# cv-core/MIT-Driverless-CV-TrainingInfra

Hardware: AMD Instinct MI355X
Metric: images/sec training (YOLOv3 416^2 + RektNet 80^2) (higher is better)
Workload: dtype bf16; 1 GPU; CVC-YOLOv3 yolo_baseline 416x416 classes=80, train step (fwd+bwd+Adam), 32 img/GPU; global_batch=32, parallelism=dp1, hipgraph=False, optimizer=FusedAdam

## Files before the change

include/mdcv_hip.h:

```cpp
#ifndef MDCV_HIP_H
#define MDCV_HIP_H
#ifdef __cplusplus
extern "C" {
#endif

#define MDCV_OK 0
#define MDCV_EARG (-1)
#define MDCV_F32 0
#define MDCV_BF16 1
#define MDCV_TUNED(dtype, code) (((dtype) & 0xff) | ((code) * 256))
#define MDCV_ACT_NONE 0
#define MDCV_ACT_LEAKY 1
#define MDCV_ACT_RELU 2

int mdcv_conv2d(int dtype, int mode, const void* in, int in_ldc, const void* w_packed, void* out, int out_ldc,
                const float* bias, const void* addsrc, int add_ldc, float* stats_partial,
                int B, int Hin, int Win, int Cin, int Hout, int Wout, int Nout,
                int KH, int KW, int stride, int pad, int dil, void* stream);
int mdcv_conv2d_affine_act(int dtype, const void* in, int in_ldc, const void* w_packed, void* out, int out_ldc, const float* scale,
                           const float* shift, const void* addsrc, int add_ldc, int act, float slope, int B, int Hin, int Win, int Cin,
                           int Hout, int Wout, int Nout, int KH, int KW, int stride, int pad, int dil, void* stream);
int mdcv_conv2d_dgrad_bnsums_rows(int dtype, int B, int Hin, int Win, int Cin, int Hout, int Wout, int Nout, int KH, int KW, int stride,
                                  int pad, int dil, int in_ldc);
int mdcv_conv2d_dgrad_bnsums(int dtype, const void* in, int in_ldc, const void* w_packed, void* out, int out_ldc, const void* addsrc,
                             int add_ldc, int B, int Hin, int Win, int Cin, int Hout, int Wout, int Nout, int KH, int KW, int stride,
                             int pad, int dil, const void* y, int ldy, const float* scale, const float* shift, const float* mean, int act,
                             float slope, float* partial, void* stream);
int mdcv_first_conv_ok(int dtype, int B, int H, int W, int Cin_pad, int Cout_pad, int KH, int KW, int stride, int pad, int dil, int ldx);
int mdcv_first_conv_rows(int B, int H);
int mdcv_first_conv_stats(int dtype, const void* x, int ldx, const void* w_packed, float* partial, int B, int H, int W, void* stream);
int mdcv_first_conv_bn_act(int dtype, const void* x, int ldx, const void* w_packed, const float* scale, const float* shift, int act, float slope,
                           void* y, int ldy, void* z, int ldz, int B, int H, int W, void* stream);
int mdcv_conv2d_dgrad_s2_form_ok(int dtype, int B, int Hin, int Win, int Cin, int Hout, int Wout, int Nout, int KH, int KW, int stride,
                                 int pad, int dil, int in_ldc);
int mdcv_xstats_words(int reps, int C);
int mdcv_xstats_reps(int rows, int C);
int mdcv_conv2d_xstats(int dtype, const void* in, int in_ldc, const void* w_packed, void* out, int out_ldc, const float* bias, void* xacc,
                       int reps, int B, int Hin, int Win, int Cin, int Hout, int Wout, int Nout, int KH, int KW, int stride, int pad, int dil,
                       void* stream);
int mdcv_pw_conv_fwd_xstats(int dtype, const void* y, int ldy, const float* scale, const float* shift, const void* resid, int ldr, int act,
                            float slope, void* z_out, int ldz, const void* w_packed, const float* bias, void* out, int out_ldc, void* xacc,
                            int reps, long long M, int K, int N, void* stream);
int mdcv_bn_act_fwd_xstats(int dtype, const void* y, int ldy, const void* xacc, int reps, double count, const float* gamma, const float* beta,
                           float* running_mean, float* running_var, float momentum, float eps, float* scale, float* shift, float* mean,
                           float* invstd, const void* resid, int ldr, void* out, int ldo, int M, int C, int act, float slope, void* stream);
int mdcv_conv2d_stats_rows(int M);
int mdcv_conv2d_stats_rows_geom(int dtype, int B, int Hout, int Wout, int Cin, int Nout, int KH, int KW, int stride, int pad, int dil,
                                int in_ldc);

int mdcv_conv2d_wgrad_splits(int dtype, int M, int Cout, int Ktot);
int mdcv_conv2d_wgrad_splits_geom(int dtype, int B, int Hin, int Win, int Cin, int Hout, int Wout, int Cout, int KH, int KW, int stride,
                                  int pad, int dil, int dy_ldc, int x_ldc);
int mdcv_conv2d_wgrad(int dtype, const void* dy, int dy_ldc, const void* x, int x_ldc, float* ws, int splits,
                      float* dw_oihw, int accumulate, int B, int Hin, int Win, int Cin, int Cin_real,
                      int Hout, int Wout, int Cout, int Cout_real, int KH, int KW, int stride, int pad, int dil, void* stream);

int mdcv_pack_weights(int dtype, const float* w_oihw, void* w_fwd, void* w_dgrad, int Cout, int Cin, int KH, int KW,
                      int Cout_pad, int Cin_pad, void* stream);

int mdcv_pack_weights_batched(int dtype, const void* table, int nlayers, int max_taps, void* stream);

int mdcv_nchw_to_nhwc(int dtype, const float* src, void* dst, int B, int C, int H, int W, int ldc, int Cpad, void* stream);
int mdcv_nhwc_to_nchw(int dtype, const void* src, int ldc, float* dst, int B, int C, int H, int W, void* stream);

int mdcv_partial_reduce(const float* partial, int rows, int nsums, int C, double* accum, void* stream);
int mdcv_bn_finalize(double* accum, double count, const float* gamma, const float* beta, float* running_mean, float* running_var,
                     float momentum, float eps, float* scale, float* shift, float* mean, float* invstd, int C, void* stream);
// ... 174 lines not shown
```

mit-driverless-cv-traininginfra_amd/csrc/conv_igemm.hip:

```cpp
#include "conv_gemm.h"
#include "conv_shift.h"
#include "wgrad_gemm.h"
#include "wgrad_shift.h"
#include "wgrad_stream.h"

extern "C" {

static int conv2d_impl(int dtype, int mode, const void* in, int in_ldc, const void* w_packed, void* out, int out_ldc,
                       const float* bias, const void* addsrc, int add_ldc, float* stats_partial,
                       int B, int Hin, int Win, int Cin, int Hout, int Wout, int Nout,
                       int KH, int KW, int stride, int pad, int dil, const BnFuseArgs* fuse, void* stream, const EpiArgs* epi = nullptr,
                       const XAccArgs* xacc = nullptr) {
  if (!in || !w_packed || !out) return MDCV_EARG;
  if (xacc && (mode != 0 || stats_partial || fuse || epi || !xacc->acc || xacc->reps < 1 || (xacc->reps & (xacc->reps - 1)))) return MDCV_EARG;
  if (epi && (mode != 0 || stats_partial || fuse)) return MDCV_EARG;
  if ((Cin & 7) || (Nout & 7) || (in_ldc & 7) || (out_ldc & 7) || (addsrc && (add_ldc & 7))) return MDCV_EARG;
  if (stride != 1 && stride != 2) return MDCV_EARG;
  if (mode != 0 && mode != 1) return MDCV_EARG;
  ConvArgs a;
  a.in = in; a.w = w_packed; a.out = out; a.bias = bias; a.addsrc = addsrc; a.stats = stats_partial;
  a.in_ldc = in_ldc; a.out_ldc = out_ldc; a.add_ldc = add_ldc;
  a.Hin = Hin; a.Win = Win; a.Cin = Cin; a.Hout = Hout; a.Wout = Wout; a.Nout = Nout;
  a.KH = KH; a.KW = KW; a.stride = stride; a.pad = pad; a.dil = dil;
  a.M = B * Hout * Wout; a.Ktot = KH * KW * Cin; a.tiles_n = 0; a.sshift = stride == 2 ? 1 : 0; a.tiles_total = 0; a.xcd_chunk = 0;
// ... 105 lines not shown
    int rows = 0;
    for (int cls = 0; cls < 4; ++cls) {
      const int ph = cls >> 1, pw = cls & 1;
      const int m = B * ((Hout - ph + 1) / 2) * ((Wout - pw + 1) / 2);
      if (m > 0) rows += cdiv(m, 128);
    }
    return rows;
  }
  return cdiv(B * Hout * Wout, 128);
}

int mdcv_conv2d_dgrad_bnsums(int dtype, const void* in, int in_ldc, const void* w_packed, void* out, int out_ldc, const void* addsrc,
                             int add_ldc, int B, int Hin, int Win, int Cin, int Hout, int Wout, int Nout, int KH, int KW, int stride,
                             int pad, int dil, const void* y, int ldy, const float* scale, const float* shift, const float* mean, int act,
                             float slope, float* partial, void* stream) {
  MDCV_TUNE_ENTRY(dtype, MDCV_TUNE_CONV);
  if (!y || !scale || !shift || !mean || !partial || (ldy & 7)) return MDCV_EARG;
  if (mdcv_conv2d_dgrad_bnsums_rows(dtype, B, Hin, Win, Cin, Hout, Wout, Nout, KH, KW, stride, pad, dil, in_ldc) <= 0) return MDCV_EARG;
  BnFuseArgs f;
  f.y = y; f.scale = scale; f.shift = shift; f.mean = mean; f.partial = partial; f.ldy = ldy; f.act = act; f.row_base = 0;
  f.slope = act == 2 ? 0.f : slope;
  return conv2d_impl(dtype, 1, in, in_ldc, w_packed, out, out_ldc, nullptr, addsrc, add_ldc, nullptr, B, Hin, Win, Cin, Hout, Wout, Nout,
                     KH, KW, stride, pad, dil, &f, stream);
}

int mdcv_conv2d_dgrad_s2_form_ok(int dtype, int B, int Hin, int Win, int Cin, int Hout, int Wout, int Nout, int KH, int KW, int stride,
                                 int pad, int dil, int in_ldc) {
  MDCV_TUNE_ENTRY(dtype, MDCV_TUNE_CONV);
  return dtype == MDCV_BF16 && stride == 2 && dil == 1 && KH == 3 && KW == 3 && pad == 1 && Hout == 2 * Hin && Wout == 2 * Win &&
         TUNE().conv_variant < 0 && (long long)B * Hin * Win * in_ldc * 2 < (1LL << 31) &&
         mdcv_shift_s2_dgrad_eligible(dtype, B, Hin, Win, Cin, Nout, in_ldc);
}

int mdcv_conv2d_stats_rows(int M) { return cdiv(M, 128); }
int mdcv_conv2d_stats_rows_geom(int dtype, int B, int Hout, int Wout, int Cin, int Nout, int KH, int KW, int stride, int pad, int dil,
                                int in_ldc) {
  MDCV_TUNE_ENTRY(dtype, MDCV_TUNE_CONV);
  if (mdcv_shift_eligible(dtype, B, Hout, Wout, Cin, Nout, KH, KW, stride, pad, dil, in_ldc)) return mdcv_shift_fwd_stats_rows(B, Hout, Wout, Nout, dil);
  return cdiv(B * Hout * Wout, 128);
}

int mdcv_conv2d_wgrad_splits(int dtype, int M, int Cout, int Ktot) {
  MDCV_TUNE_ENTRY(dtype, MDCV_TUNE_WGRAD);
  const int bp = dtype == MDCV_BF16 ? 128 : 64;
  const int tiles = cdiv(Cout, 128) * cdiv(Ktot, 128);
  const int slots = TUNE().wgrad_slots;
  int s = slots / tiles;
  const int max_s = cdiv(M, bp * 4);
  if (s > max_s) s = max_s;
  if (s < 1) s = 1;
  int pps = cdiv(cdiv(M, s), bp) * bp;
  return cdiv(M, pps);
}

enum WgradFamily { WG_STEM, WG_STREAM, WG_SHIFT, WG_S2, WG_GENERIC };

static bool wgrad_eligible(WgradFamily f, const WgradGeom& g) {
  const int v = TUNE().wgrad_variant;
  if (f == WG_GENERIC) return true;
  if (v == 9 || (v == 10 && f != WG_SHIFT)) return false;
  const bool same = g.Hin == g.Hout && g.Win == g.Wout;
  switch (f) {
    case WG_STEM:
      return same && mdcv_wgrad_stem_eligible(g.dtype, g.B, g.Hout, g.Wout, g.Cin, g.Cout, g.KH, g.KW, g.stride, g.pad, g.dil, g.dy_ldc, g.x_ldc);
    case WG_STREAM:
      return same && mdcv_wgrad_stream_eligible(g.dtype, g.B, g.Hout, g.Wout, g.Cin, g.Cout, g.KH, g.KW, g.stride, g.pad, g.dil, g.dy_ldc, g.x_ldc);
// ... 92 lines not shown
```

mit-driverless-cv-traininginfra_amd/csrc/conv_shift.h:

```cpp
#pragma once
#include <hip/hip_runtime.h>
#include "bn_fuse.h"
#include "exact_acc.h"

struct ShiftArgs {
  const void* in; const void* w; void* out; const float* bias; const void* addsrc; float* stats;
  int in_ldc, out_ldc, add_ldc;
  int B, H, W, Cin, Nout;
  int Wq, Sq, Mq;
  int tiles_n, tiles_total, xcd_chunk;
  int p_base;
  int dil;
  BnFuseArgs fuse;
  EpiArgs epi;
  int t2d, tiles_x, tiles_y, TH;
  int nchunks, wrow, nca;
  XAccArgs xacc;
};

bool mdcv_shift_eligible(int dtype, int B, int H, int W, int Cin, int Nout, int KH, int KW, int stride, int pad, int dil, long long in_ldc);
int mdcv_shift_stats_rows(int B, int H, int W, int dil = 1, int Nout = 128);
int mdcv_shift_fwd_stats_rows(int B, int H, int W, int Nout, int dil = 1);
int mdcv_shift_conv(int mode, const void* in, int in_ldc, const void* w, void* out, int out_ldc, const float* bias, const void* addsrc,
                    int add_ldc, float* stats, int B, int H, int W, int Cin, int Nout, const BnFuseArgs* fuse, hipStream_t st,
                    const EpiArgs* epi = nullptr, int dil = 1, const XAccArgs* xacc = nullptr);
int mdcv_shift_s2_rows(int B, int H, int W);
bool mdcv_shift_s2_dgrad_eligible(int dtype, int B, int H, int W, int Cin, int Nout, long long in_ldc);
```

mit-driverless-cv-traininginfra_amd/csrc/conv_shift.hip:

```cpp
#include "common.h"
#include "conv_shift.h"
#include "bn_fuse.h"

#ifndef MDCV_SHIFT_PART
#define MDCV_SHIFT_PART 0
#endif
#if MDCV_SHIFT_PART == 0
#else
#endif
int mdcv_shift_launch_dgrad(const ShiftArgs& a, hipStream_t st, unsigned in_bytes, unsigned w_bytes);

namespace {

[[maybe_unused]] constexpr int BN = 128;
constexpr int WM = 4;
constexpr unsigned OOB = 0x80000000u;

__device__ __forceinline__ int swz(int row) { return (row >> 1) & 2; }
typedef __attribute__((address_space(3))) void lds_void_t;

#if defined(MDCV_SHIFT_TS) || defined(MDCV_SHIFT_WG)
#include <cstdio>
__device__ long long g_shift_wg[3 * 4096];
#endif
#ifdef MDCV_SHIFT_TS
__device__ long long g_shift_ts[4 * 512];
#define STS(k) do { if (ts_on && ts_i < 512) g_shift_ts[(k) * 512 + ts_i] = (long long)clock64(); } while (0)
#else
#define STS(k)
#endif

template <int N> __device__ __forceinline__ void wait_vm() { asm volatile("s_waitcnt vmcnt(%0)" ::"n"(N) : "memory"); }
template <int N> __device__ __forceinline__ void wait_vm_reads_done() { asm volatile("s_waitcnt vmcnt(%0) lgkmcnt(0)" ::"n"(N) : "memory"); }

}

template <int MODE, int BM, int NPA, int BRING, bool FUSE, int WN, bool EPI = false, int BN_ = 128, int LOOP = 0>
__global__ __launch_bounds__(WM * WN * 64) void mdcv_conv3x3_shift_kernel(ShiftArgs a, unsigned in_bytes, unsigned w_bytes) {
  constexpr int BN = BN_, BTILE = BN * 64, SROW = BN * 2 + 16;
  constexpr int NW = WM * WN, TN = BN / WN, FN = TN / 16;
  constexpr int TM = BM / WM, FM = TM / 16;
  static_assert(!FUSE || (WN == 2 && BM % 128 == 0), "the fused sums: 8 waves, one partial row per 128 positions");
  constexpr int STAGE = BM * SROW;
  constexpr int PIX_OFF = STAGE;
  constexpr int STAT_OFF = STAGE + BM * 4;
  extern __shared__ __attribute__((aligned(1024))) unsigned char smem[];
  const int ABYTES = a.nca * 1024;
  const int BBASE = 2 * ABYTES;
  const int SINK = BBASE + BRING * BTILE;

  const int logical = (int)(blockIdx.x & 7) * a.xcd_chunk + (int)(blockIdx.x >> 3);
  if (logical >= a.tiles_total) return;
  const int tid = threadIdx.x, lane = tid & 63;
  const int wave = __builtin_amdgcn_readfirstlane(tid >> 6);
  const int wm = wave / WN, wn = wave % WN;
  const int tile_m = logical / a.tiles_n, tile_n = logical % a.tiles_n;
  const int p0 = a.p_base + tile_m * BM;
  const int lrow = lane >> 2, kv = (lane & 3) ^ swz(lrow);

  unsigned avo[NPA];
#pragma unroll
  for (int k = 0; k < NPA; ++k) {
    const int j = (wave + k * NW) * 16 + lrow;
    int img, yy, xx;
    bool ok;
    if (a.t2d) {
      const int tpi = a.tiles_x * a.tiles_y;
      img = tile_m / tpi;
      const int rt = tile_m - img * tpi, ty = rt / a.tiles_x, tx = rt - ty * a.tiles_x;
      const int cy = j / a.Wq, cx = j - cy * a.Wq;
// ... 38 lines not shown
    const int so__ = (CHUNK) * 64;                                                                                  \
    _Pragma("unroll") for (int k = 0; k < NPA; ++k) {                                                               \
      const int ch__ = wave + k * NW;              \
      __builtin_amdgcn_raw_ptr_buffer_load_lds(RS, (lds_void_t*)(smem + (ch__ < a.nca ? base__ + ch__ * 1024 : SINK)), 16, \
                                               (int)avo[k], so__, 0, 0);                                            \
    }                                                                                                               \
  } while (0)
#define ISSUE_B(RS, TAP, CHUNK, SLOT)                                                                               \
  __builtin_amdgcn_raw_ptr_buffer_load_lds(RS, (lds_void_t*)(smem + (wave < BN / 16 ? BBASE + (SLOT) * BTILE + wave * 1024 : SINK)), 16, (int)bvo, \
                                           ((TAP) * a.Cin + (CHUNK) * 32) * 2, 0, 0)

  constexpr int NCLS = MODE == 3 ? 4 : 1;
#define TAP_CLS(T) (MODE == 3 ? ((((T) / 3) != 1 ? 2 : 0) + (((T) % 3) != 1 ? 1 : 0)) * FM : 0)
  f32x4_t acc[NCLS * FM][FN];
#pragma unroll
  for (int i = 0; i < NCLS * FM; ++i)
#pragma unroll
    for (int j = 0; j < FN; ++j) acc[i][j] = f32x4_t{0.f, 0.f, 0.f, 0.f};

  constexpr int LA = BRING - 1;
  const int nch = a.nchunks;
#ifdef MDCV_SHIFT_TS
  const bool ts_on = logical == 300 && tid == 64 * 3;
  int ts_i = 0;
#endif
#if defined(MDCV_SHIFT_TS) || defined(MDCV_SHIFT_WG)
  if (tid == 0 && logical < 4096) {
    g_shift_wg[logical] = (long long)wall_clock64();
    unsigned hwid; asm volatile("s_getreg_b32 %0, hwreg(HW_REG_HW_ID)" : "=s"(hwid));
    unsigned xcc; asm volatile("s_getreg_b32 %0, hwreg(HW_REG_XCC_ID)" : "=s"(xcc));
    g_shift_wg[2 * 4096 + logical] = (long long)hwid | ((long long)xcc << 32);
  }
#endif
  ISSUE_A(rin, 0, 0);
#pragma unroll
  for (int t = 0; t < LA; ++t) ISSUE_B(rw, t % 9, t / 9, t);
  constexpr int PERIOD = BRING == 4 ? 4 : 2;
  static_assert((9 * PERIOD) % BRING == 0, "ring period");
  if constexpr (LOOP == 1) {
    const int grp = wave >> 2;
    wait_vm<LA - 1>();
    __builtin_amdgcn_s_barrier();
    if (grp == 1) __builtin_amdgcn_s_barrier();
    for (int c0 = 0; c0 < nch; c0 += PERIOD) {
#pragma unroll
      for (int cc = 0; cc < PERIOD; ++cc) {
        const int c = c0 + cc;
        if (c < nch) {
          const bool lastc = c == nch - 1;
          const int abase = (cc & 1) * ABYTES;
#pragma unroll
          for (int tap = 0; tap < 9; ++tap) {
            const int rslot = (cc * 9 + tap) % BRING, wslot = (cc * 9 + tap + LA) % BRING;
            bf16x8_t fa[FM], fb[FN];
            const unsigned char* pa = smem + abase + offA[tap];
            const unsigned char* pb = smem + BBASE + rslot * BTILE + offB;
#pragma unroll
            for (int j = 0; j < FN; ++j) fb[j] = *reinterpret_cast<const bf16x8_t*>(pb + j * 1024);
#pragma unroll
            for (int i = 0; i < FM; ++i) fa[i] = *reinterpret_cast<const bf16x8_t*>(pa + i * 1024);
            {
              const int t2 = (tap + LA) % 9, c2 = c + (tap + LA) / 9;
              if (tap + LA >= 9 && lastc) ISSUE_B(rw0, t2, c2, wslot);
              else ISSUE_B(rw, t2, c2, wslot);
            }
            if (tap == 0) {
              if (lastc) ISSUE_A(rin0, c + 1, (cc + 1) & 1);
              else ISSUE_A(rin, c + 1, (cc + 1) & 1);
            }
            if (tap <= LA - 1) wait_vm_reads_done<LA - 1 + NPA>(); else wait_vm_reads_done<LA - 1>();
#pragma unroll
            for (int i = 0; i < FM; ++i) asm volatile("" : "+v"(fa[i]));
// ... 58 lines not shown
#pragma unroll
          for (int i = 0; i < FM; ++i)
#pragma unroll
            for (int j = 0; j < FN; ++j) acc[TAP_CLS(tap) + i][j] = __builtin_amdgcn_mfma_f32_16x16x32_bf16(fa[i], fb[j], acc[TAP_CLS(tap) + i][j], 0, 0, 0);
#ifdef MDCV_SHIFT_PRIO
          __builtin_amdgcn_s_setprio(0);
#endif
          STS(3);
#ifdef MDCV_SHIFT_TS
          ++ts_i;
#endif
        }
      }
    }
  }
  }
  wait_vm<0>();
  __syncthreads();

  if constexpr (MODE == 3) {
    static_assert(MODE != 3 || (BM == 256 && !EPI), "stride-2 data gradient: 8 x 32 dY positions per tile");
    const int tpi = a.tiles_x * a.tiles_y;
    const int img = tile_m / tpi, rt = tile_m - img * tpi, ty = rt / a.tiles_x, tx = rt - ty * a.tiles_x;
    const int a0 = ty * a.TH, b0 = tx * (a.Wq - 1);
    const int Ho = 2 * a.H, Wo = 2 * a.W;
    bf16_t* __restrict__ out3 = reinterpret_cast<bf16_t*>(a.out);
    const bf16_t* __restrict__ add3 = reinterpret_cast<const bf16_t*>(a.addsrc);
    constexpr int VPRO3 = BN / 8;
    static_assert((512 * VPRO3) % (NW * 64) == 0 && (NW * 64) % VPRO3 == 0, "every thread keeps one channel vector");
    using Acc3 = BnFuseAcc<bf16_t, BN, NW * 64>;
    Acc3 fz3;
    const bf16_t* __restrict__ fy3 = reinterpret_cast<const bf16_t*>(a.fuse.y);
    if constexpr (FUSE) fz3.init(a.fuse, tile_n * BN + (tid % VPRO3) * 8, a.Nout);
#pragma unroll
    for (int py = 0; py < 2; ++py) {
#pragma unroll
      for (int px = 0; px < 2; ++px)
#pragma unroll
        for (int i = 0; i < FM; ++i)
#pragma unroll
          for (int j = 0; j < FN; ++j)
#pragma unroll
            for (int rr = 0; rr < 4; ++rr) {
              const int p = wm * TM + i * 16 + (lane >> 4) * 4 + rr, col = wn * TN + j * 16 + (lane & 15);
              const int srow = (p >> 5) * 64 + 2 * (p & 31) + px;
              reinterpret_cast<bf16_t*>(smem + srow * SROW)[col] = f2bf(acc[(2 * py + px) * FM + i][j][rr]);
            }
      __syncthreads();
      long long pixv[VPRO3]; uint4 aq[VPRO3], yq[VPRO3];
      const int cv = tid % VPRO3, n = tile_n * BN + cv * 8;
#pragma unroll
      for (int k = 0; k < VPRO3; ++k) {
        const int srow = (tid + k * NW * 64) / VPRO3;
        const int la = srow >> 6, ox = srow & 63;
        const int Y = 2 * (a0 + la) + py, X = 2 * b0 + ox;
        const bool ok = ox < 2 * (a.Wq - 1) && Y < Ho && X < Wo && n < a.Nout;
        pixv[k] = ok ? ((long long)img * Ho + Y) * Wo + X : -1;
        if (ok) {
          if (add3) aq[k] = *reinterpret_cast<const uint4*>(add3 + pixv[k] * a.add_ldc + n);
          if constexpr (FUSE) yq[k] = *reinterpret_cast<const uint4*>(fy3 + pixv[k] * a.fuse.ldy + n);
        }
      }
#pragma unroll
      for (int k = 0; k < VPRO3; ++k) {
        if (pixv[k] >= 0) {
          const int srow = (tid + k * NW * 64) / VPRO3;
          uint4 d = *reinterpret_cast<const uint4*>(smem + srow * SROW + cv * 16);
          float x[8];
          if (add3 || FUSE) ET<bf16_t>::unpack(d, x);
          if (add3) {
            float y[8];
            ET<bf16_t>::unpack(aq[k], y);
#pragma unroll
            for (int e = 0; e < 8; ++e) x[e] += y[e];
            d = ET<bf16_t>::pack(x);
            if constexpr (FUSE) ET<bf16_t>::unpack(d, x);
          }
          if constexpr (FUSE) {
            fz3.add(a.fuse, x, yq[k]);
          }
          *reinterpret_cast<uint4*>(out3 + pixv[k] * a.out_ldc + n) = d;
        }
      }
      __syncthreads();
    }
    if constexpr (FUSE) {
      static_assert(Acc3::kWaveFold, "bf16, at most 16 channel vectors per pixel");
      float* ws3 = reinterpret_cast<float*>(smem + 512 * SROW);
      fz3.fold_wave(ws3 + wave * 2 * BN, lane);
      lds_only_barrier();
      for (int t = tid; t < 2 * BN; t += NW * 64) Acc3::write_row(a.fuse, ws3, 2 * BN, t, tile_n * BN, a.Nout, tile_m);
    }
    return;
  }
  int* rowpix = reinterpret_cast<int*>(smem + PIX_OFF);
  if (tid < BM) {
    int img, y, x;
    bool ok;
    if (a.t2d) {
      const int tpi = a.tiles_x * a.tiles_y;
      img = tile_m / tpi;
      const int rt = tile_m - img * tpi, ty = rt / a.tiles_x, tx = rt - ty * a.tiles_x;
      const int ly = tid / a.Wq, lx = tid - ly * a.Wq;
      y = ty * a.TH + ly; x = tx * (a.Wq - 2) + lx;
      ok = lx < a.Wq - 2 && ly < a.TH;
    } else {
      const int p = p0 + tid;
      ok = p < a.Mq;
      const int pp = ok ? p : 0;
      img = pp / a.Sq;
      const int rem = pp - img * a.Sq;
      y = rem / a.Wq; x = rem - y * a.Wq;
    }
    ok = ok && y < a.H && x < a.W;
    rowpix[tid] = ok ? (img * a.H + y) * a.W + x : -1;
  }
  const int n0 = tile_n * BN + wn * TN;
// ... 143 lines not shown
#pragma unroll
            for (int e = 0; e < 8; ++e) x[e] += y[e];
            d = ET<bf16_t>::pack(x);
            ET<bf16_t>::unpack(d, x);
          }
          *reinterpret_cast<uint4*>(out + ((size_t)pixv[gi][u] * a.out_ldc + n)) = d;
          fz.add(a.fuse, x, yq[gi][u]);
        }
      }
      if (p0 + g0 < a.Mq) {
        if constexpr (Acc::kWaveFold)
          fz.fold_wave(reinterpret_cast<float*>(smem + (g0 + wave * Acc::WROWS) * SROW), lane);
        else
          fz.flush(a.fuse, fred, tid, tile_n * BN, a.Nout, (p0 + g0) >> 7);
      }
    }
    if constexpr (Acc::kWaveFold) {
      static_assert(Acc::WROWS * SROW >= 2 * BN * 4 && SROW % 4 == 0, "a wave's dead staging rows hold its 2*BN sums");
      lds_only_barrier();
      for (int t = tid; t < NG * 2 * BN; t += NW * 64) {
        const int gi = t / (2 * BN), g0 = gi * 128;
        if (p0 + g0 < a.Mq)
          Acc::write_row(a.fuse, reinterpret_cast<const float*>(smem + g0 * SROW), Acc::WROWS * SROW / 4, t - gi * 2 * BN, tile_n * BN, a.Nout, (p0 + g0) >> 7);
      }
    }
  }
#if defined(MDCV_SHIFT_TS) || defined(MDCV_SHIFT_WG)
  if (tid == 0 && logical < 4096) g_shift_wg[4096 + logical] = (long long)wall_clock64();
#endif
}

namespace {

template <int MODE, int BM, int NPA, bool FUSE, int WN, bool EPI = false, int BRING = 3, int BN_ = 128, int LOOP = 0>
int launch_shift_f(ShiftArgs a, int p_base, int tiles_m, hipStream_t st, unsigned in_bytes, unsigned w_bytes) {
  constexpr int NW = WM * WN;
  constexpr int BN = BN_, BTILE = BN * 64, SROW = BN * 2 + 16;
  if constexpr (LOOP == 0 && WN == 2 && !EPI && MODE == 0 && !FUSE) {
    if (TUNE().shift_loop == 1 || BM > 256 || (TUNE().shift_loop == 2 && tiles_m * a.tiles_n <= 256))
      return launch_shift_f<MODE, BM, NPA, FUSE, WN, EPI, BRING, BN_, 1>(a, p_base, tiles_m, st, in_bytes, w_bytes);
  }
  if constexpr (BRING == 3 && WN == 2 && !EPI) {
    if ((TUNE().shift_ring == 4 && tiles_m * a.tiles_n <= 256) || TUNE().shift_ring == 5)
      return launch_shift_f<MODE, BM, NPA, FUSE, WN, EPI, 4, BN_, LOOP>(a, p_base, tiles_m, st, in_bytes, w_bytes);
  }
  a.p_base = p_base;
  a.tiles_total = tiles_m * a.tiles_n;
  a.xcd_chunk = (a.tiles_total + 7) / 8;
  a.nca = (BM + 2 * a.dil * (a.Wq + 1) + 15) / 16;
  const int pipe = 2 * a.nca * 1024 + BRING * BTILE + 1024;
  const int epi = MODE == 3 ? 512 * SROW + NW * 2 * BN * 4
                            : BM * SROW + BM * 4 + WM * 2 * BN * 4;
  const int lds = pipe > epi ? pipe : epi;
  static DynLds dyn_lds;
  auto kern = mdcv_conv3x3_shift_kernel<MODE, BM, NPA, BRING, FUSE, WN, EPI, BN_, LOOP>;
  if (hipError_t e = mdcv_dyn_lds(dyn_lds, reinterpret_cast<const void*>(kern), lds); e != hipSuccess) return (int)e;
  MDCV_LAUNCH(kern, dim3((unsigned)(a.xcd_chunk * 8)), dim3(NW * 64), lds, st, a, in_bytes, w_bytes);
  MDCV_CHECK_LAUNCH();
  return MDCV_OK;
}

template <int MODE, int BM, int NPA, int WN, int BN_>
int launch_shift(const ShiftArgs& a, int p_base, int tiles_m, hipStream_t st, unsigned in_bytes, unsigned w_bytes) {
  if constexpr (MODE == 3) {
    if (a.fuse.y) return launch_shift_f<MODE, BM, NPA, true, WN, false, 3, BN_>(a, p_base, tiles_m, st, in_bytes, w_bytes);
  }
  if constexpr (MODE == 1 && WN == 2 && BM % 128 == 0) {
    if (a.fuse.y) return launch_shift_f<MODE, BM, NPA, true, WN, false, 3, BN_>(a, p_base, tiles_m, st, in_bytes, w_bytes);
  }
  if constexpr (MODE == 0 && WN == 2) {
    if (a.epi.oscale || a.epi.act) return launch_shift_f<MODE, BM, NPA, false, WN, true, 3, BN_>(a, p_base, tiles_m, st, in_bytes, w_bytes);
  }
  if (a.epi.oscale || a.epi.act) return MDCV_EARG;
  return launch_shift_f<MODE, BM, NPA, false, WN, false, 3, BN_>(a, p_base, tiles_m, st, in_bytes, w_bytes);
}

template <int MODE, int BM, int BN_>
int launch_shift_bm(const ShiftArgs& a, int p_base, int tiles_m, hipStream_t st, unsigned in_bytes, unsigned w_bytes) {
  const int nca = (BM + 2 * a.dil * (a.Wq + 1) + 15) / 16;
  const int npa = (nca + 7) / 8;
  if (npa <= 2) return launch_shift<MODE, BM, 2, 2, BN_>(a, p_base, tiles_m, st, in_bytes, w_bytes);
  if (npa == 3) return launch_shift<MODE, BM, 3, 2, BN_>(a, p_base, tiles_m, st, in_bytes, w_bytes);
  if (npa == 4) return launch_shift<MODE, BM, 4, 2, BN_>(a, p_base, tiles_m, st, in_bytes, w_bytes);
  return launch_shift<MODE, BM, 5, 2, BN_>(a, p_base, tiles_m, st, in_bytes, w_bytes);
}

int shift_plan_bm(int Mq, int tiles_n, bool fused, int halo = 0, int bn = 128, bool fwd = false) {
  if (halo > 0 && !fused && 2 * ((256 + halo + 15) / 16) * 1024 + 3 * bn * 64 + 1024 > 80 * 1024) {
// ... 52 lines not shown
  if (a.Nout == 32) return launch_shift_mode<1, 32>(a, st, in_bytes, w_bytes);
  if (a.Nout == 64) return launch_shift_mode<1, 64>(a, st, in_bytes, w_bytes);
  if (TUNE().shift_n64_wide && !a.t2d && a.Nout % 64 == 0 && ((a.Mq + 255) / 256) * a.tiles_n <= 128) {
    ShiftArgs b = a;
    b.tiles_n = a.Nout / 64;
    return launch_shift_mode<1, 64>(b, st, in_bytes, w_bytes);
  }
  return launch_shift_mode<1, 128>(a, st, in_bytes, w_bytes);
}
#else
static bool shift_fits_1d(int W, int Nout) {
  return W <= TUNE().shift_wmax || (TUNE().shift_wmax_narrow && Nout <= 64 && W <= TUNE().shift_wmax_narrow) || (TUNE().shift_wmax_n32 && Nout <= 32 && W <= TUNE().shift_wmax_n32);
}
static bool shift_is_2d(int W, int Nout, int dil) { return dil == 1 && TUNE().shift_2d && !shift_fits_1d(W, Nout); }
constexpr int T2D_WQ = 32, T2D_TH = 8;
static long long shift_2d_positions(int B, int H, int W) { return (long long)B * ((H + T2D_TH - 1) / T2D_TH) * ((W + T2D_WQ - 3) / (T2D_WQ - 2)) * 256; }

bool mdcv_shift_eligible(int dtype, int B, int H, int W, int Cin, int Nout, int KH, int KW, int stride, int pad, int dil, long long in_ldc) {
  if (dtype != MDCV_BF16 || KH != 3 || KW != 3 || stride != 1 || pad != dil || (dil != 1 && !(dil == 2 && TUNE().shift_dil2))) return false;
  if (dil == 2 && TUNE().shift_dil2 == 1 && !(Nout <= 64 && Cin >= 64)) return false;
  if ((Cin & 31) || ((Nout & 127) && !(Nout == 64 && TUNE().shift_n64) && !(Nout == 32 && TUNE().shift_n64 == 2))) return false;
  if (H < 8 || W < 8) return false;
  if (!shift_fits_1d(W, Nout) && !(TUNE().shift_2d && dil == 1)) return false;
  if ((long long)B * (H + dil) * (W + dil) + 1024 >= (1LL << 30) || shift_2d_positions(B, H, W) >= (1LL << 30)) return false;
  if ((long long)B * H * W * in_ldc * 2 >= (1LL << 31) || (long long)Nout * 9 * Cin * 2 >= (1LL << 31)) return false;
  return true;
}

bool mdcv_shift_s2_dgrad_eligible(int dtype, int B, int H, int W, int Cin, int Nout, long long in_ldc) {
  if (!TUNE().shift_s2 || dtype != MDCV_BF16 || (Cin & 31) || Cin < 32 || !(Nout == 32 || Nout == 64) || H < 1 || W < 1) return false;
  if ((long long)B * ((H + 7) / 8) * ((W + 30) / 31) * 256 >= (1LL << 30)) return false;
  if ((long long)B * H * W * in_ldc * 2 >= (1LL << 31) || (long long)Nout * 9 * Cin * 2 >= (1LL << 31)) return false;
  return true;
}

int mdcv_shift_s2_rows(int B, int H, int W) { return B * ((H + T2D_TH - 1) / T2D_TH) * ((W + T2D_WQ - 2) / (T2D_WQ - 1)); }

int mdcv_shift_stats_rows(int B, int H, int W, int dil, int Nout) {
  if (shift_is_2d(W, Nout, dil)) return (int)(shift_2d_positions(B, H, W) / 128);
  return (int)(((long long)B * (H + dil) * (W + dil) + 127) / 128);
}
int mdcv_shift_fwd_stats_rows(int B, int H, int W, int Nout, int dil) {
  if (shift_is_2d(W, Nout, dil)) return (int)(shift_2d_positions(B, H, W) / 128);
  const int Mq = B * (H + dil) * (W + dil);
  const int bn = Nout <= 64 ? Nout : BN;
  const int bm = shift_plan_bm(Mq, Nout <= 64 ? 1 : Nout / BN, false, 2 * dil * (W + dil + 1), bn, true);
  return (bm == 192 || bm == 384) ? (Mq + bm - 1) / bm : (Mq + 127) / 128;
}

int mdcv_shift_conv(int mode, const void* in, int in_ldc, const void* w, void* out, int out_ldc, const float* bias, const void* addsrc,
                    int add_ldc, float* stats, int B, int H, int W, int Cin, int Nout, const BnFuseArgs* fuse, hipStream_t st,
                    const EpiArgs* epi, int dil, const XAccArgs* xacc) {
  ShiftArgs a;
  a.xacc = XAccArgs{nullptr, 1};
  if (xacc) { if (mode != 0 || stats || epi || !xacc->acc || xacc->reps < 1 || (xacc->reps & (xacc->reps - 1))) return MDCV_EARG; a.xacc = *xacc; }
  if (fuse) a.fuse = *fuse; else a.fuse = BnFuseArgs{};
  if (epi) a.epi = *epi; else a.epi = EpiArgs{nullptr, 0, 0.f};
  a.in = in; a.w = w; a.out = out; a.bias = bias; a.addsrc = addsrc; a.stats = stats;
  a.in_ldc = in_ldc; a.out_ldc = out_ldc; a.add_ldc = add_ldc;
  a.B = B; a.H = H; a.W = W; a.Cin = Cin; a.Nout = Nout;
  a.dil = dil; a.Wq = W + dil; a.Sq = (H + dil) * (W + dil); a.Mq = B * a.Sq;
  a.t2d = 0; a.tiles_x = a.tiles_y = a.TH = 0;
  if (mode == 3) {
    a.t2d = 2; a.Wq = T2D_WQ; a.TH = T2D_TH;
    a.tiles_x = (W + T2D_WQ - 2) / (T2D_WQ - 1); a.tiles_y = (H + T2D_TH - 1) / T2D_TH;
    a.Mq = B * a.tiles_x * a.tiles_y * 256; a.Sq = a.tiles_x * a.tiles_y * 256;
// ... 41 lines not shown
```

mit-driverless-cv-traininginfra_amd/csrc/tune.h:

```cpp
#pragma once

struct MdcvTune {
  int conv_no_ut = 0;
  int conv_tall_narrow = 256;
  int conv_deep_narrow = 1;
  int conv_deep_small = 8;
  int conv_fuse_narrow = 1;
  int conv_variant = -1;
  int conv_tall_s2 = 1;
  int conv_deep_s2 = 1;
  int conv_s2_allcls = 1;
  int conv_s2_split = 512;
  int conv_s2_split_on = 1;
  int wgrad_slots = 512;
  int wgrad_bna_stages = 2;
  int wgrad_variant = 0;
  int shift_ring = 4;
  int shift_wmax_narrow = 104;
  int shift_wmax_n32 = 0;
  int shift_dil2 = 1;
  int shift_n64 = 2;
  int shift_wmax = 80;
  int shift_loop = 2;
  int shift_2d = 1;
  int shift_big = 0;
  int shift_n64_wide = 1;
  int shift_plan = 0;
  int shift_s2 = 1;
  int pw_bmp = 0;
  int pw_wres = 1;
  int stream_blocks = 0;
  int stream_tiled = 1;
  int stream_light_maxpos = 600000;
  int stream_table = 1;
  int stream_direct = 1;
  int stream_s2 = 1;
  int stream_s2_blocks = 256;
  int stream_s2_depth = 2;
  int stream_s2_lds = 160 * 1024;
  int stream_light_depth = 1;
  int stream_light_blocks = 256;
  int stream_tiled_blocks = 128;
};

extern thread_local const MdcvTune* mdcv_t_tune;
inline const MdcvTune& TUNE() { return *mdcv_t_tune; }

enum { MDCV_TUNE_CONV = 0, MDCV_TUNE_WGRAD = 1, MDCV_TUNE_PW = 2 };

inline void mdcv_tune_shift(MdcvTune& t, int ring) {
  if (ring == 63 || ring == 64) { t.shift_n64_wide = ring - 63; return; }
  if (ring == 29 || ring == 60) { t.shift_s2 = ring == 60; return; }
  if (ring == 27 || ring == 28) { t.shift_2d = ring - 27; return; }
  if (ring >= 200 && ring < 300) { t.shift_big = ring == 201 ? 384 : 0; return; }
  if (ring >= 30 && ring <= 59) { t.shift_loop = ring - 30; return; }
  if (ring == 25 || ring == 26) { t.shift_wmax_n32 = ring == 25 ? 208 : 0; return; }
  if (ring == 23 || ring == 24) { t.shift_wmax_narrow = ring == 23 ? 104 : 0; return; }
  if (ring >= 20 && ring <= 22) { t.shift_dil2 = ring == 20 ? 2 : (ring == 21 ? 0 : 1); return; }
  if (ring >= 17 && ring <= 19) { t.shift_n64 = ring == 17 ? 1 : (ring == 18 ? 0 : 2); return; }
  if (ring >= 14 && ring <= 16) { t.shift_wmax = ring == 14 ? 80 : (ring == 15 ? 62 : 104); return; }
  if (ring >= 7) t.shift_plan = ring - 7;
  else if (ring >= 3 && ring <= 5) t.shift_ring = ring;
}
inline void mdcv_tune_apply_conv(MdcvTune& t, int v) {
  if (v == 0) return;
  if (v <= -3 && v >= -299) { mdcv_tune_shift(t, -v); return; }
  if (v == 93 || v == 92) { t.conv_fuse_narrow = v == 93; return; }
  if (v >= 60 && v < 92) { t.conv_deep_small = v - 60; return; }
  if (v >= 30 && v < 60) { t.conv_deep_narrow = v - 30; return; }
  if (v == 20 || v == 21) { t.conv_deep_s2 = v - 20; return; }
  if (v == 16 || v == 17) { t.conv_s2_allcls = v - 16; return; }
  if (v == 14 || v == 15) { t.conv_s2_split_on = v - 14; return; }
  if (v >= 4000 && v < 6000) { t.conv_s2_split = v - 4000; return; }
  if (v == 18 || v == 19) { t.conv_tall_s2 = v - 18; return; }
  if (v >= 2000 && v < 3000) { t.conv_tall_narrow = v - 2000; return; }
  if (v >= 100) { t.conv_no_ut = 1; v -= 100; }
  if (v >= 1 && v <= 12) t.conv_variant = v - 1;
}
inline void mdcv_tune_apply_wgrad(MdcvTune& t, int v) {
  if (v == 0) return;
  if (v >= 20000 && v < 30000) { t.wgrad_slots = v - 20000; return; }
  if (v >= 35000 && v < 36000) { t.stream_s2_blocks = v - 35000; return; }
  if (v >= 30000 && v < 40000) {
// ... 43 lines not shown
```

Before: 2489 images/sec.

## Add tap-grouped weight pipelining loop for narrow shift convs and optional s2 epilogue

Adds a new main-loop variant (LOOP==2) for the 3x3 shift convolution kernel with narrow output tiles (32/64 channels): weights for groups of 3 or 9 taps are staged into LDS per barrier with double buffering, so there are fewer barriers per input-channel chunk. The variant is on by default when the LDS budget allows, and a query function is exported for callers. A separate stride-2 dgrad epilogue that prefetches residual and BN operands is added behind a tune flag that is off by default. The change adds LDS pressure and more template instantiations, and it could lower occupancy for the affected layers.

```diff
diff --git a/include/mdcv_hip.h b/include/mdcv_hip.h
--- a/include/mdcv_hip.h
+++ b/include/mdcv_hip.h
@@ -33,6 +33,8 @@
                            void* y, int ldy, void* z, int ldz, int B, int H, int W, void* stream);
 int mdcv_conv2d_dgrad_s2_form_ok(int dtype, int B, int Hin, int Win, int Cin, int Hout, int Wout, int Nout, int KH, int KW, int stride,
                                  int pad, int dil, int in_ldc);
+int mdcv_conv2d_shift_tapgroup(int dtype, int mode, int B, int Hin, int Win, int Cin, int Hout, int Wout, int Nout, int KH, int KW, int stride,
+                               int pad, int dil, int in_ldc);
 int mdcv_xstats_words(int reps, int C);
 int mdcv_xstats_reps(int rows, int C);
 int mdcv_conv2d_xstats(int dtype, const void* in, int in_ldc, const void* w_packed, void* out, int out_ldc, const float* bias, void* xacc,
diff --git a/mit-driverless-cv-traininginfra_amd/csrc/conv_igemm.hip b/mit-driverless-cv-traininginfra_amd/csrc/conv_igemm.hip
--- a/mit-driverless-cv-traininginfra_amd/csrc/conv_igemm.hip
+++ b/mit-driverless-cv-traininginfra_amd/csrc/conv_igemm.hip
@@ -161,6 +161,19 @@
          mdcv_shift_s2_dgrad_eligible(dtype, B, Hin, Win, Cin, Nout, in_ldc);
 }
 
+int mdcv_conv2d_shift_tapgroup(int dtype, int mode, int B, int Hin, int Win, int Cin, int Hout, int Wout, int Nout, int KH, int KW, int stride,
+                               int pad, int dil, int in_ldc) {
+  MDCV_TUNE_ENTRY(dtype, MDCV_TUNE_CONV);
+  if (TUNE().conv_variant >= 0 || (mode != 0 && mode != 1)) return 0;
+  if (!conv_operands_small((long long)B * Hin * Win * in_ldc * 2, (long long)Nout * KH * KW * Cin * 2)) return 0;
+  if (mode == 1 && stride == 2)
+    return dil == 1 && KH == 3 && KW == 3 && pad == 1 && Hout == 2 * Hin && Wout == 2 * Win && mdcv_shift_s2_dgrad_eligible(dtype, B, Hin, Win, Cin, Nout, in_ldc)
+               ? mdcv_shift_tapgroup(3, Win, Cin, Nout, 1) : 0;
+  if (Hin == Hout && Win == Wout && mdcv_shift_eligible(dtype, B, Hout, Wout, Cin, Nout, KH, KW, stride, pad, dil, in_ldc))
+    return mdcv_shift_tapgroup(mode, Wout, Cin, Nout, dil);
+  return 0;
+}
+
 int mdcv_conv2d_stats_rows(int M) { return cdiv(M, 128); }
 int mdcv_conv2d_stats_rows_geom(int dtype, int B, int Hout, int Wout, int Cin, int Nout, int KH, int KW, int stride, int pad, int dil,
                                 int in_ldc) {
diff --git a/mit-driverless-cv-traininginfra_amd/csrc/conv_shift.h b/mit-driverless-cv-traininginfra_amd/csrc/conv_shift.h
--- a/mit-driverless-cv-traininginfra_amd/csrc/conv_shift.h
+++ b/mit-driverless-cv-traininginfra_amd/csrc/conv_shift.h
@@ -26,3 +26,4 @@
                     const EpiArgs* epi = nullptr, int dil = 1, const XAccArgs* xacc = nullptr);
 int mdcv_shift_s2_rows(int B, int H, int W);
 bool mdcv_shift_s2_dgrad_eligible(int dtype, int B, int H, int W, int Cin, int Nout, long long in_ldc);
+int mdcv_shift_tapgroup(int mode, int W, int Cin, int Nout, int dil = 1);
diff --git a/mit-driverless-cv-traininginfra_amd/csrc/conv_shift.hip b/mit-driverless-cv-traininginfra_amd/csrc/conv_shift.hip
--- a/mit-driverless-cv-traininginfra_amd/csrc/conv_shift.hip
+++ b/mit-driverless-cv-traininginfra_amd/csrc/conv_shift.hip
@@ -35,7 +35,7 @@
 
 }
 
-template <int MODE, int BM, int NPA, int BRING, bool FUSE, int WN, bool EPI = false, int BN_ = 128, int LOOP = 0>
+template <int MODE, int BM, int NPA, int BRING, bool FUSE, int WN, bool EPI = false, int BN_ = 128, int LOOP = 0, int TG = 0, bool S2E = false>
 __global__ __launch_bounds__(WM * WN * 64) void mdcv_conv3x3_shift_kernel(ShiftArgs a, unsigned in_bytes, unsigned w_bytes) {
   constexpr int BN = BN_, BTILE = BN * 64, SROW = BN * 2 + 16;
   constexpr int NW = WM * WN, TN = BN / WN, FN = TN / 16;
@@ -140,12 +140,88 @@
     g_shift_wg[2 * 4096 + logical] = (long long)hwid | ((long long)xcc << 32);
   }
 #endif
-  ISSUE_A(rin, 0, 0);
-#pragma unroll
-  for (int t = 0; t < LA; ++t) ISSUE_B(rw, t % 9, t / 9, t);
+  if constexpr (LOOP != 2) {
+    ISSUE_A(rin, 0, 0);
+#pragma unroll
+    for (int t = 0; t < LA; ++t) ISSUE_B(rw, t % 9, t / 9, t);
+  }
   constexpr int PERIOD = BRING == 4 ? 4 : 2;
   static_assert((9 * PERIOD) % BRING == 0, "ring period");
-  if constexpr (LOOP == 1) {
+  if constexpr (LOOP == 2) {
+    static_assert(TG == 3 || TG == 9, "taps per barrier");
+    static_assert(BN <= 64 && NW % (BN / 16) == 0, "narrow tiles: every wave keeps one 16-row piece of the weight tile");
+    constexpr int GPC = 9 / TG, GB = TG * BTILE;
+    constexpr int WPT = BN / 16, TPR = NW / WPT, NPB = (TG + TPR - 1) / TPR;
+    const int BB2 = (nch * GPC == 1 ? 1 : 2) * ABYTES;
+    const int bsub = wave % WPT, bt0 = wave / WPT;
+    unsigned bvo2;
+    {
+      const int n = tile_n * BN + bsub * 16 + lrow;
+      bvo2 = n < a.Nout ? (unsigned)((n * a.wrow + kv * 8) * 2) : OOB;
+    }
+#define ISSUE_A2(CHUNK, BUF)                                                                                          \
+  do {                                                                                                              \
+    _Pragma("unroll") for (int k = 0; k < NPA; ++k) {                                                               \
+      const int ch__ = wave + k * NW;                                                                               \
+      if (ch__ < a.nca)                                                                                             \
+        __builtin_amdgcn_raw_ptr_buffer_load_lds(rin, (lds_void_t*)(smem + (BUF) * ABYTES + ch__ * 1024), 16, (int)avo[k], (CHUNK) * 64, 0, 0); \
+    }                                                                                                               \
+  } while (0)
+#define ISSUE_BG(TAP0, CHUNK, BUF)                                                                                    \
+  do {                                                                                                              \
+    _Pragma("unroll") for (int k = 0; k < NPB; ++k) {                                                               \
+      const int t__ = bt0 + k * TPR;                                                                                \
+      if (t__ < TG)                                                                                                 \
+        __builtin_amdgcn_raw_ptr_buffer_load_lds(rw, (lds_void_t*)(smem + BB2 + (BUF) * GB + t__ * BTILE + bsub * 1024), 16, (int)bvo2, \
+                                                 (((TAP0) + t__) * a.Cin + (CHUNK) * 32) * 2, 0, 0);                \
+    }                                                                                                               \
+  } while (0)
+    ISSUE_A2(0, 0);
+    ISSUE_BG(0, 0, 0);
+    wait_vm_reads_done<0>();
+    for (int c0 = 0; c0 < nch; c0 += 2) {
+#pragma unroll
+      for (int cc = 0; cc < 2; ++cc) {
+        const int c = c0 + cc;
+        if (c < nch) {
+          const bool lastc = c == nch - 1;
+          const int abase = cc * ABYTES;
+#pragma unroll
+          for (int gi = 0; gi < GPC; ++gi) {
+            const int gbuf = (cc * GPC + gi) & 1;
+            __builtin_amdgcn_s_barrier();
+            if (gi + 1 < GPC) ISSUE_BG((gi + 1) * TG, c, gbuf ^ 1);
+            else if (!lastc) {
+              ISSUE_BG(0, c + 1, gbuf ^ 1);
+              ISSUE_A2(c + 1, cc ^ 1);
+            }
+#pragma unroll
+            for (int tl = 0; tl < TG; ++tl) {
+              const int tap = gi * TG + tl;
+              bf16x8_t fa[FM], fb[FN];
+              const unsigned char* pa = smem + abase + offA[tap];
+              const unsigned char* pb = smem + BB2 + gbuf * GB + tl * BTILE + offB;
+#pragma unroll
+              for (int i = 0; i < FM; ++i) fa[i] = *reinterpret_cast<const bf16x8_t*>(pa + i * 1024);
+#pragma unroll
+              for (int j = 0; j < FN; ++j) fb[j] = *reinterpret_cast<const bf16x8_t*>(pb + j * 1024);
+#pragma unroll
+              for (int i = 0; i < FM; ++i)
+#pragma unroll
+                for (int j = 0; j < FN; ++j) acc[TAP_CLS(tap) + i][j] = __builtin_amdgcn_mfma_f32_16x16x32_bf16(fa[i], fb[j], acc[TAP_CLS(tap) + i][j], 0, 0, 0);
+            }
+#pragma unroll
+            for (int i = 0; i < NCLS * FM; ++i)
+#pragma unroll
+              for (int j = 0; j < FN; ++j) asm volatile("" : "+v"(acc[i][j]));
+            wait_vm_reads_done<0>();
+          }
+        }
+      }
+    }
+#undef ISSUE_A2
+#undef ISSUE_BG
+  } else if constexpr (LOOP == 1) {
     const int grp = wave >> 2;
     wait_vm<LA - 1>();
     __builtin_amdgcn_s_barrier();
@@ -270,6 +346,69 @@
     Acc3 fz3;
     const bf16_t* __restrict__ fy3 = reinterpret_cast<const bf16_t*>(a.fuse.y);
     if constexpr (FUSE) fz3.init(a.fuse, tile_n * BN + (tid % VPRO3) * 8, a.Nout);
+    if constexpr (S2E) {
+      static_assert(BN == 32, "see launch_shift_f");
+      constexpr bool HB = FUSE, PF1 = HB;
+      long long pixv[2][VPRO3]; uint4 aq[2][VPRO3], yq[2][VPRO3];
+      const int cv = tid % VPRO3, n = tile_n * BN + cv * 8;
+#define S2_OPERANDS(PY)                                                                                               \
+  _Pragma("unroll") for (int k = 0; k < VPRO3; ++k) {                                                               \
+    const int srow = (tid + k * NW * 64) / VPRO3;                                                                   \
+    const int la = srow >> 6, ox = srow & 63;                                                                       \
+    const int Y = 2 * (a0 + la) + (PY), X = 2 * b0 + ox;                                                            \
+    const bool ok = ox < 2 * (a.Wq - 1) && Y < Ho && X < Wo && n < a.Nout;                                          \
+    pixv[PY][k] = ok ? ((long long)img * Ho + Y) * Wo + X : -1;                                                     \
+    if (ok) {                                                                                                       \
+      if (add3) aq[PY][k] = *reinterpret_cast<const uint4*>(add3 + pixv[PY][k] * a.add_ldc + n);                    \
+      if constexpr (FUSE) yq[PY][k] = *reinterpret_cast<const uint4*>(fy3 + pixv[PY][k] * a.fuse.ldy + n);          \
+    }                                                                                                               \
+  }
+      if constexpr (HB) { S2_OPERANDS(0); }
+#pragma unroll
+      for (int py = 0; py < 2; ++py) {
+        if (py == 1 && HB && !PF1) { S2_OPERANDS(1); }
+#pragma unroll
+        for (int px = 0; px < 2; ++px)
+#pragma unroll
+          for (int i = 0; i < FM; ++i)
+#pragma unroll
+            for (int j = 0; j < FN; ++j)
+#pragma unroll
+              for (int rr = 0; rr < 4; ++rr) {
+                const int p = wm * TM + i * 16 + (lane >> 4) * 4 + rr, col = wn * TN + j * 16 + (lane & 15);
+                const int srow = (p >> 5) * 64 + 2 * (p & 31) + px;
+                reinterpret_cast<bf16_t*>(smem + srow * SROW)[col] = f2bf(acc[(2 * py + px) * FM + i][j][rr]);
+              }
+        if (!HB) {
+          if (py == 0) { S2_OPERANDS(0); } else { S2_OPERANDS(1); }
+        }
+        lds_only_barrier();
+        if (py == 0 && PF1) { S2_OPERANDS(1); }
+#pragma unroll
+        for (int k = 0; k < VPRO3; ++k) {
+          if (pixv[py][k] >= 0) {
+            const int srow = (tid + k * NW * 64) / VPRO3;
+            uint4 d = *reinterpret_cast<const uint4*>(smem + srow * SROW + cv * 16);
+            float x[8];
+            if (add3 || FUSE) ET<bf16_t>::unpack(d, x);
+            if (add3) {
+              float y[8];
+              ET<bf16_t>::unpack(aq[py][k], y);
+#pragma unroll
+              for (int e = 0; e < 8; ++e) x[e] += y[e];
+              d = ET<bf16_t>::pack(x);
+              if constexpr (FUSE) ET<bf16_t>::unpack(d, x);
+            }
+            if constexpr (FUSE) {
+              fz3.add(a.fuse, x, yq[py][k]);
+            }
+            *reinterpret_cast<uint4*>(out3 + pixv[py][k] * a.out_ldc + n) = d;
+          }
+        }
+        if (py == 0) lds_only_barrier();
+      }
+#undef S2_OPERANDS
+    } else {
 #pragma unroll
     for (int py = 0; py < 2; ++py) {
 #pragma unroll
@@ -321,6 +460,7 @@
         }
       }
       __syncthreads();
+    }
     }
     if constexpr (FUSE) {
       static_assert(Acc3::kWaveFold, "bf16, at most 16 channel vectors per pixel");
@@ -530,28 +670,52 @@
 
 namespace {
 
-template <int MODE, int BM, int NPA, bool FUSE, int WN, bool EPI = false, int BRING = 3, int BN_ = 128, int LOOP = 0>
+inline int shift_tapgroup_tg(bool s2, int bn, int nchunks, int nca) {
+  const int srow = bn * 2 + 16;
+  const int epi = s2 ? 512 * srow + WM * 2 * 2 * bn * 4 : 256 * srow + 256 * 4 + WM * 2 * bn * 4;
+  for (int tg = 9; tg >= 3; tg -= 6) {
+    const int nb = nchunks * (9 / tg) == 1 ? 1 : 2;
+    const int pipe = nb * (nca * 1024 + tg * bn * 64);
+    if ((pipe > epi ? pipe : epi) <= 80 * 1024) return tg;
+  }
+  return 0;
+}
+
+template <int MODE, int BM, int NPA, bool FUSE, int WN, bool EPI = false, int BRING = 3, int BN_ = 128, int LOOP = 0, int TG = 0, bool S2E = false>
 int launch_shift_f(ShiftArgs a, int p_base, int tiles_m, hipStream_t st, unsigned in_bytes, unsigned w_bytes) {
   constexpr int NW = WM * WN;
   constexpr int BN = BN_, BTILE = BN * 64, SROW = BN * 2 + 16;
+  if constexpr (MODE == 3 && NPA == 3 && BN_ == 32 && !S2E) {
+    if (TUNE().shift_s2_epi) return launch_shift_f<MODE, BM, NPA, FUSE, WN, EPI, BRING, BN_, LOOP, TG, true>(a, p_base, tiles_m, st, in_bytes, w_bytes);
+  }
+  if constexpr (LOOP == 0 && BN_ <= 64 && WN == 2 && !EPI && BM == 256 && NPA == 3 && BRING == 3) {
+    if (TUNE().shift_tapgroup && a.t2d) {
+      const int tg = shift_tapgroup_tg(MODE == 3, BN_, a.nchunks, (BM + 2 * a.dil * (a.Wq + 1) + 15) / 16);
+      if (tg == 9) return launch_shift_f<MODE, BM, NPA, FUSE, WN, EPI, BRING, BN_, 2, 9, S2E>(a, p_base, tiles_m, st, in_bytes, w_bytes);
+      if constexpr (BN_ == 64) {
+        if (tg == 3) return launch_shift_f<MODE, BM, NPA, FUSE, WN, EPI, BRING, BN_, 2, 3, S2E>(a, p_base, tiles_m, st, in_bytes, w_bytes);
+      }
+    }
+  }
   if constexpr (LOOP == 0 && WN == 2 && !EPI && MODE == 0 && !FUSE) {
     if (TUNE().shift_loop == 1 || BM > 256 || (TUNE().shift_loop == 2 && tiles_m * a.tiles_n <= 256))
-      return launch_shift_f<MODE, BM, NPA, FUSE, WN, EPI, BRING, BN_, 1>(a, p_base, tiles_m, st, in_bytes, w_bytes);
-  }
-  if constexpr (BRING == 3 && WN == 2 && !EPI) {
+      return launch_shift_f<MODE, BM, NPA, FUSE, WN, EPI, BRING, BN_, 1, TG, S2E>(a, p_base, tiles_m, st, in_bytes, w_bytes);
+  }
+  if constexpr (BRING == 3 && WN == 2 && !EPI && LOOP != 2) {
     if ((TUNE().shift_ring == 4 && tiles_m * a.tiles_n <= 256) || TUNE().shift_ring == 5)
-      return launch_shift_f<MODE, BM, NPA, FUSE, WN, EPI, 4, BN_, LOOP>(a, p_base, tiles_m, st, in_bytes, w_bytes);
+      return launch_shift_f<MODE, BM, NPA, FUSE, WN, EPI, 4, BN_, LOOP, TG, S2E>(a, p_base, tiles_m, st, in_bytes, w_bytes);
   }
   a.p_base = p_base;
   a.tiles_total = tiles_m * a.tiles_n;
   a.xcd_chunk = (a.tiles_total + 7) / 8;
   a.nca = (BM + 2 * a.dil * (a.Wq + 1) + 15) / 16;
-  const int pipe = 2 * a.nca * 1024 + BRING * BTILE + 1024;
+  const int nbuf = a.nchunks * 9 == TG ? 1 : 2;
+  const int pipe = LOOP == 2 ? nbuf * (a.nca * 1024 + TG * BTILE) : 2 * a.nca * 1024 + BRING * BTILE + 1024;
   const int epi = MODE == 3 ? 512 * SROW + NW * 2 * BN * 4
                             : BM * SROW + BM * 4 + WM * 2 * BN * 4;
   const int lds = pipe > epi ? pipe : epi;
   static DynLds dyn_lds;
-  auto kern = mdcv_conv3x3_shift_kernel<MODE, BM, NPA, BRING, FUSE, WN, EPI, BN_, LOOP>;
+  auto kern = mdcv_conv3x3_shift_kernel<MODE, BM, NPA, BRING, FUSE, WN, EPI, BN_, LOOP, TG, S2E>;
   if (hipError_t e = mdcv_dyn_lds(dyn_lds, reinterpret_cast<const void*>(kern), lds); e != hipSuccess) return (int)e;
   MDCV_LAUNCH(kern, dim3((unsigned)(a.xcd_chunk * 8)), dim3(NW * 64), lds, st, a, in_bytes, w_bytes);
   MDCV_CHECK_LAUNCH();
@@ -670,6 +834,11 @@
   if ((long long)B * ((H + 7) / 8) * ((W + 30) / 31) * 256 >= (1LL << 30)) return false;
   if ((long long)B * H * W * in_ldc * 2 >= (1LL << 31) || (long long)Nout * 9 * Cin * 2 >= (1LL << 31)) return false;
   return true;
+}
+
+int mdcv_shift_tapgroup(int mode, int W, int Cin, int Nout, int dil) {
+  if (!TUNE().shift_tapgroup || !(Nout == 32 || Nout == 64) || (mode != 3 && !shift_is_2d(W, Nout, dil))) return 0;
+  return shift_tapgroup_tg(mode == 3, Nout, (Cin + 31) / 32, (256 + 2 * (T2D_WQ + 1) + 15) / 16);
 }
 
 int mdcv_shift_s2_rows(int B, int H, int W) { return B * ((H + T2D_TH - 1) / T2D_TH) * ((W + T2D_WQ - 2) / (T2D_WQ - 1)); }
diff --git a/mit-driverless-cv-traininginfra_amd/csrc/tune.h b/mit-driverless-cv-traininginfra_amd/csrc/tune.h
--- a/mit-driverless-cv-traininginfra_amd/csrc/tune.h
+++ b/mit-driverless-cv-traininginfra_amd/csrc/tune.h
@@ -27,6 +27,8 @@
   int shift_n64_wide = 1;
   int shift_plan = 0;
   int shift_s2 = 1;
+  int shift_tapgroup = 1;
+  int shift_s2_epi = 0;
   int pw_bmp = 0;
   int pw_wres = 1;
   int stream_blocks = 0;
@@ -49,6 +51,9 @@
 enum { MDCV_TUNE_CONV = 0, MDCV_TUNE_WGRAD = 1, MDCV_TUNE_PW = 2 };
 
 inline void mdcv_tune_shift(MdcvTune& t, int ring) {
+  if (ring == 65 || ring == 66) { t.shift_tapgroup = ring - 65; return; }
+  if (ring == 67 || ring == 68) { t.shift_s2_epi = ring - 67; return; }
+  if (ring >= 69 && ring <= 71) { t.shift_tapgroup = ring == 70; t.shift_s2_epi = ring != 69; return; }
   if (ring == 63 || ring == 64) { t.shift_n64_wide = ring - 63; return; }
   if (ring == 29 || ring == 60) { t.shift_s2 = ring == 60; return; }
   if (ring == 27 || ring == 28) { t.shift_2d = ring - 27; return; }
```

Result: no change. 2491 images/sec, median of 2 (+0.1%).
